# f1tenth/f1tenth_gym

Hardware: AMD Instinct MI355X
Metric: agent-steps/s (1080-beam scan + ST dynamics) (higher is better)
Workload: dtype f64

## Files before the change

### f1tenth_gym_amd/csrc/f110_hip.hip

```cpp
#include <hip/hip_runtime.h>
#include <rccl/rccl.h>

#include <dlfcn.h>

#include <algorithm>
#include <chrono>
#include <cmath>
#include <cstdarg>
#include <cstdio>
#include <cstdlib>
#include <cstring>
#include <map>
#include <mutex>
#include <new>
#include <set>
#include <string>
#include <vector>

#include "../../include/f110.h"
#include "f110_kernels.hpp"
#include "f110_devmem.hpp"

using devmem::DevArena;
using devmem::DevBuf;
// ... 2590 lines not shown
    double *d = reinterpret_cast<double *>(base + ((ints * 4 + 63) / 64) * 64);
    t.state = d;            d += 7 * N;
    t.steer_buf = d;        d += 2 * N;
    t.scan_pose = d;        d += 3 * N;
    t.snap_pose = d;        d += 3 * N;
    t.dir_start = d;        d += N;
    t.ray_hdr = reinterpret_cast<RayHdr *>(d);
    t.tasks_per_agent = ((uint32_t)h->k.num_beams + 63u) / 64u;
    return F110_OK;
}

static int step_tiny(f110_sim *h, hipStream_t st, const double *d_actions, const StepRequest &rq, bool &host_written)
{
    TRY(tiny_setup(h));
    const int N = h->N, A = h->cfg.num_agents;
    AgentArrays dev = h->dev;
    dev.agent_begin = 0;
    dev.agent_count = N;
    dev.sched_count_zero = nullptr;
    RayJob j{};
    j.noise = h->dev.noise;
    j.ttc_side_max = h->ttc_side_max;
    j.ttc_k = h->dev.ttc_thresh * (1.0 + 1e-9) * h->ttc_cos_max;
    j.beam_cos = h->dev.beam_cos;
    j.side_dist = h->dev.side_dist;
    j.ttc_thresh = h->dev.ttc_thresh;
    j.k_cold = cold_consts(h);
    if (!j.k_cold) return fail(h, F110_ERR_HIP, "f110_step_device: constant upload failed");
    h->tiny.tasks_per_agent = ((uint32_t)h->k.num_beams + 63u) / 64u;
    h->tiny.trace = kExperimental ? reinterpret_cast<unsigned long long *>(h->exp.tiny_trace) : nullptr;
    h->tiny.act_inline = 0;
    if (rq.tiny_actions && N <= kTinyMaxAgents) {
        std::memcpy(h->tiny.act, rq.tiny_actions, sizeof(double) * 2 * (size_t)N);
        h->tiny.act_inline = 1;
    }
    h->tiny.start_word = nullptr;
    h->tiny.skip = kExperimental ? (h->exp.tiny_start_probe == 2 ? 1 : (h->exp.tiny_general_tail ? 2 : 0)) : 0;
    if (kExperimental && h->exp.tiny_start_probe && h->hb_seq_host && rq.seq) {
        void *p = nullptr;
        TRY(map_host_ptr(h, h->hb_seq_host, &p, "completion word"));
        h->tiny.start_word = reinterpret_cast<unsigned long long *>(p) + 1;
        h->tiny.start_seq = h->hb_seq;
    }
    const dim3 grid(((unsigned)N * h->tiny.tasks_per_agent + 3u) / 4u), block(256);
    const bool host = !dev.reseat_poses && (A == 2 ? rq.fuse : rq.hb != nullptr), solo = host && A != 2;
    host_written = host;
// ... 12 lines not shown
    if (A == 2) {
        if (host) { if (ident) TINY(true, true, true); else TINY(true, false, true); }
        else { if (ident) TINY(true, true, false); else TINY(true, false, false); }
    } else {
        if (host) { if (ident) TINY(false, true, true); else TINY(false, false, true); }
        else { if (ident) TINY(false, true, false); else TINY(false, false, false); }
    }
#undef TINY
    h->last_launches = 1;
    if (h->track_on) {
        TRY(track_launch(h, st, kTrackPost, 0, N));
        h->last_launches += 2;
    }
    return F110_OK;
}

static int step_range(f110_sim *h, hipStream_t st, int begin, int count, const double *d_actions, int collide_mode, hipEvent_t *ev, const StepRequest &rq,
                      bool &host_written)
{
    const int N = h->N, A = h->cfg.num_agents, B = h->k.num_beams;
    AgentArrays dev = h->dev;
    dev.agent_begin = begin;
    dev.agent_count = count;
    const bool multi = A > 1;
    const ScanKind scan = pick_scan(h, begin, count);
    if (h->track_on) TRY(track_launch(h, st, kTrackHead, begin, count));
    dev.sched_count_zero = scan == SCAN_AGENT_SCHED ? h->d_tcount + (h->task_epoch & 1u) : nullptr;
    if (dev.noise_rng && (dev.noise_rng == 2 || h->noise_ub >= (long long)dev.noise_rows)) {
        const int apb = dev.noise_rng == 2 ? 16 : 64;
        hipLaunchKernelGGL(k_noise_rows, dim3((count + apb - 1) / apb), dim3(256), 0, st, dev, h->noise_gen, B, apb);
    }
    if (ev) HIPCHK(h, hipEventRecord(ev[0], st));
    bool fused_integrate = false;
#ifdef F110_EXPERIMENTAL
    if (multi && collide_mode == 1 && A == 2) {
        hipLaunchKernelGGL(k_integrate<2>, grid1d(count, 64), dim3(64), 0, st, dev, h->k, d_actions);
        fused_integrate = true;
    } else if (multi && collide_mode == 1 && A == 4) {
        hipLaunchKernelGGL(k_integrate<4>, grid1d(count, 64), dim3(64), 0, st, dev, h->k, d_actions);
        fused_integrate = true;
    }
#endif
    if (!fused_integrate) {
        bool duo = true;
        bool fan = h->dev.integrator == F110_INTEGRATOR_RK4 && count <= kFanMaxAgents;
#ifdef F110_EXPERIMENTAL
// ... 10 lines not shown
    const bool multi_in_finalize = multi && collide_mode == 3 && A > 2 && A <= kMaxAgentsMulti && (begin % A) == 0 && (count % A) == 0;
    const bool no_collide_launch = fused_integrate || pair_in_finalize || multi_in_finalize;
    const bool side_collide = multi && !no_collide_launch && !(kExperimental && collide_mode == 2);
    if (multi && !no_collide_launch) {
        if (side_collide) {
            HIPCHK(h, hipEventRecord(h->ev_integrated, st));
            HIPCHK(h, hipStreamWaitEvent(h->side_stream, h->ev_integrated, 0));
            hipLaunchKernelGGL(k_collide, grid1d(count, 64), dim3(64), 0, h->side_stream, dev, B);
            HIPCHK(h, hipEventRecord(h->ev_collided, h->side_stream));
        } else {
            hipLaunchKernelGGL(k_collide, grid1d(count, 64), dim3(64), 0, st, dev, B);
        }
    }
    if (ev) HIPCHK(h, hipEventRecord(ev[1], st));
    {
        RayJob j{};
        j.n_rays = (uint32_t)N * (uint32_t)B;
        j.n_poses = N;
        j.pose_x = h->dev.scan_pose;
        j.pose_y = h->dev.scan_pose + N;
        j.dir_start = h->dev.dir_start;
        j.ranges = h->dev.scans;
        j.hdr = h->dev.ray_hdr;
        j.noise = h->dev.noise;
        j.ttc_side_max = h->ttc_side_max;
        j.ttc_k = h->dev.ttc_thresh * (1.0 + 1e-9) * h->ttc_cos_max;
        j.beam_cos = h->dev.beam_cos;
        j.side_dist = h->dev.side_dist;
        j.wall_flag = h->dev.in_collision;
        j.ttc_thresh = h->dev.ttc_thresh;
        j.div_magic = h->step_magic;
        j.div_shift = h->step_shift;
        j.lookups_total = h->lookups_on ? h->d_lookups : nullptr;
        j.path_stats = h->path_stats_on ? h->d_path_stats : nullptr;
#ifdef F110_EXPERIMENTAL
        j.trace = reinterpret_cast<unsigned long long *>(h->exp.scan_trace);
#endif
        j.k_cold = cold_consts(h);
        if (!j.k_cold) return fail(h, F110_ERR_HIP, "f110_step_device: constant upload failed");
        j.order = (h->multi_map && begin == 0 && count == N) ? h->d_scan_order : nullptr;
        const bool cnt = j.lookups_total != nullptr;
        const bool env_order = h->scan_env_order && !h->multi_map && (scan == SCAN_AGENT || scan == SCAN_AGENT_SCHED);
        auto agent_grid = [&](uint32_t tpa, dim3 &grid, uint32_t &wpb, int tpw) {
            (void)rays_grid(j, h->scan_block, tpw);
            j.n_tasks = (uint32_t)count * tpa;
            j.first_pose = (uint32_t)begin;
            j.agents_per_env = (env_order && A > 1 && begin % A == 0 && count % A == 0 && scan_task_inv_ok(tpa, (uint32_t)A)) ? (uint32_t)A : 1u;
            j.agents_inv = scan_task_inv(j.agents_per_env);
            wpb = (uint32_t)h->scan_block / 64u;
// ... 3170 lines not shown
```

### f1tenth_gym_amd/csrc/f110_kernels.hpp

```cpp
#pragma once

#include <hip/hip_runtime.h>
#include <stdint.h>

#include "f110_math.hpp"
#include "f110_rng.hpp"

using namespace f110;

struct RayHdr {
    double x, y;
    double start;
    double vel;
    double d0;
    int32_t noise_row;
    int32_t map_slot;
    int32_t pad_hdr;
    int32_t i0;
    int32_t n_dirs;
    int32_t fast;
};
static_assert(sizeof(RayHdr) == 64, "RayHdr is read as 16-byte scalar loads");

struct AgentArrays {
    int32_t n_agents_total;
    int32_t agents_per_env;
    int32_t agent_begin, agent_count;
    double *state;
    double *steer_buf;
    int32_t *buf_cnt;
    double *scan_pose;
    double *snap_pose;
    double *dir_start;
    RayHdr *ray_hdr;
    double *scans;
    double *collisions;
// ... 3 lines not shown
    unsigned long long *path_stats;
    const ScanConst *maps_full;
    const int32_t *env_map;
    const double *reseat_poses;
    int32_t *reseat_count;
    int32_t reseat_ego, pad_reseat;
    uint32_t *sched_count_zero;
    int32_t *opp_window;
    double *opp_verts;
    const double *params;
    int32_t params_per_agent, pad_params;
    const double *noise;
    int32_t noise_rng, pad_rng;
    U128 *rng_state;
    const U128 *rng_seed;
    const U128 *rng_rowstate;
    U128 rng_inc;
    const double *scan_angles, *beam_cos, *side_dist;
    int32_t noise_rows, integrator;
    double time_step, lidar_dist, ttc_thresh, angle_inc;
    double box_length, box_width;
    const struct FusedHost *fused_host;
    unsigned long long fused_seq;
};

__device__ __forceinline__ VehicleParams load_params(const double *p)
{
    VehicleParams vp;
#pragma unroll
    for (int i = 0; i < NPARAMS; ++i) vp.v[i] = p[i];
    return vp;
}

struct EpisodeArrays {
    int32_t ego_idx, pad;
    double timestep;
    double *start_poses;
    double *rot;
    double *current_time;
    uint8_t *near_start;
    double *toggle;
    double *lap_count;
    double *lap_time;
    uint8_t *done;
    uint8_t *checkpoint;
};
// ... 89 lines not shown
        }
        int ref_lo, ref_hi, lo, hi;
        box_vertices(ox, oy, oth, blen, bwid, other);
        int32_t *win = a.opp_window + ((size_t)i * A + j) * 4;
        opponent_beam_window(mx, my, mth, other, ox, oy, disc_r, a.scan_angles, B, a.angle_inc, ref_lo, ref_hi, lo, hi);
        win[0] = lo;
        win[1] = hi;
        opponent_beam_window(mx, my, 0.0, other, ox, oy, disc_r, a.scan_angles, B, a.angle_inc, ref_lo, ref_hi, lo, hi);
        win[2] = lo;
        win[3] = hi;
        double *ov = a.opp_verts + ((size_t)i * A + j) * 8;
#pragma unroll
        for (int c = 0; c < 8; ++c) ov[c] = other[c];
    }
    a.collisions[i] = hit ? 1.0 : 0.0;
    a.collision_idx[i] = (double)partner;
}

__device__ __forceinline__ RayHdr make_ray_hdr(const AgentArrays &a, const ScanConst &k, int i, const double *st, const double *sp, double start)
{
    RayHdr hd;
    ScanConst kr = k;
    kr.table = k.table_rm;
    hd.x = sp[0];
    hd.y = sp[1];
    hd.start = start;
    hd.vel = st[3];
    hd.map_slot = a.env_map ? a.env_map[i / a.agents_per_env] : 0;
    hd.pad_hdr = 0;
    const ScanConst *km = a.env_map ? a.maps_full + hd.map_slot : &kr;
    int r0, c0;
    hd.d0 = sample_distance<LAYOUT_ROWMAJOR, false, false>(*km, nullptr, sp[0], sp[1], r0, c0);
    int row = -1;
    if (a.noise_rng) {
        row = a.step_count[i];
        if (a.noise_rng == 2 || row >= a.noise_rows) row = -2;
    } else if (a.noise_rows > 0) {
        row = a.step_count[i];
        if (row >= a.noise_rows) row %= a.noise_rows;
    }
    hd.noise_row = row;
    hd.i0 = beam_dir_index(k, start, 0);
    hd.fast = 0;
    if (km->pad) {
        double ux, uy;
        padded_position<false>(*km, sp[0], sp[1], ux, uy);
        hd.fast = padded_start_ok(*km, ux, uy) ? 1 : 0;
    }
    hd.n_dirs = 0;
    if (k.theta_inc < 1.0) {
        int span = beam_dir_index(k, start, k.num_beams - 1) - hd.i0;
        if (span < 0) span += k.theta_dis;
        hd.n_dirs = span + 1;
    }
    return hd;
}

__device__ __forceinline__ void integrate_store_columns(const AgentArrays &a, int i, int N, const double *st, double b0, double b1, int cnt, const double *sp,
                                                        double start)
{
#pragma unroll
    for (int c = 0; c < 7; ++c) a.state[(size_t)c * N + i] = st[c];
    a.steer_buf[i] = b0;
    a.steer_buf[(size_t)N + i] = b1;
    a.buf_cnt[i] = cnt;
    a.scan_pose[i] = sp[0];
    a.scan_pose[(size_t)N + i] = sp[1];
    a.scan_pose[2 * (size_t)N + i] = sp[2];
    a.snap_pose[i] = st[0];
    a.snap_pose[(size_t)N + i] = st[1];
// ... 207 lines not shown
    uint32_t *count_w;
    uint32_t cap, thr;
    const void *reserved_r[8];
    uint32_t reserved_rcap, reserved_rthr;
};

struct RayJob {
    uint32_t n_rays;
    uint32_t n_tasks;
    uint32_t tasks_per_wave;
    int32_t n_poses;
    uint32_t div_magic, div_shift;
    int32_t pad_dir, dir_stride;
    const void *reserved_dir_ranges;
    uint32_t first_pose, agents_per_env;
    unsigned long long *lookups_total;
    TaskSched sched;
    uint32_t epoch_r, epoch_w, long_blocks, agents_inv;
    uint32_t *env_done;
    uint32_t tasks_per_env, long_prio;
    uint32_t long_rev, pad_rev;
    unsigned long long *trace;
    const uint32_t *order;
    const void *reserved_win[2];
    uint32_t reserved_win_pitch, pad_win;
    const double *pose_x, *pose_y, *dir_start;
    double *ranges;
    const RayHdr *hdr;
    const double *noise;
    const double *beam_cos, *side_dist;
    int32_t *wall_flag;
    double ttc_thresh;
    double ttc_side_max, ttc_k;
    int32_t *hit_rc;
    unsigned long long *lookups;
    unsigned long long *path_stats;
    const ScanConst *k_cold;
};

__device__ __forceinline__ int uniform_i32(int v) { return __builtin_amdgcn_readfirstlane(v); }
__device__ __forceinline__ double uniform_f64(double v)
{
    const int lo = __builtin_amdgcn_readfirstlane(__double2loint(v));
    const int hi = __builtin_amdgcn_readfirstlane(__double2hiint(v));
    return __hiloint2double(hi, lo);
}

struct LaneHdr {
    double x, y, start, vel, d0;
    int row, map_slot, i0, n_dirs, fast;
};

__device__ __forceinline__ LaneHdr load_lane_hdr(const RayHdr *hdr, uint32_t p)
{
    LaneHdr o;
    const uint32_t p0 = __builtin_amdgcn_readfirstlane(p);
    if (__ballot(p != p0) == 0ull) {
        typedef const __attribute__((address_space(4))) RayHdr *chdr_t;
        const chdr_t h0 = (chdr_t)(hdr) + p0;
        o.x = uniform_f64(h0->x);
        o.y = uniform_f64(h0->y);
        o.start = uniform_f64(h0->start);
        o.vel = uniform_f64(h0->vel);
        o.d0 = uniform_f64(h0->d0);
        o.row = uniform_i32(h0->noise_row);
        o.map_slot = uniform_i32(h0->map_slot);
        o.i0 = uniform_i32(h0->i0);
        o.n_dirs = uniform_i32(h0->n_dirs);
        o.fast = uniform_i32(h0->fast);
    } else {
        const RayHdr hd = hdr[p];
        o.x = hd.x; o.y = hd.y; o.start = hd.start; o.vel = hd.vel; o.d0 = hd.d0; o.row = hd.noise_row;
        o.map_slot = hd.map_slot; o.i0 = hd.i0; o.n_dirs = hd.n_dirs;
        o.fast = hd.fast;
    }
    return o;
}

struct RayJob;
__device__ __forceinline__ void finish_beam(const RayJob &j, uint32_t B, uint32_t p, int b, uint32_t ray, double r,
                                            int row, double vel);
__device__ __forceinline__ void finish_beam_with(const RayJob &j, uint32_t p, int b, uint32_t ray, double r, double vel);

__device__ __forceinline__ void wave_add_lookups(unsigned long long *total, uint32_t mine)
{
    for (int off = 32; off; off >>= 1) mine += __shfl_xor(mine, off);
    if ((threadIdx.x & 63u) == 0u) atomicAdd(total, (unsigned long long)mine);
}

template <int LAYOUT, bool POW2, bool IDENT, bool WANT_CELL>
__device__ __forceinline__ double trace_from_first(const ScanConst &k, const ScanConst *k_cold, const double *lut, double x, double y,
                                                   bool fast, double c, double s, double d0, int &hr, int &hc, int &nl,
                                                   int &path)
{
    if (LAYOUT == LAYOUT_PADDED) {
        double r = 0.;
        bool exact = !fast;
        if (fast) {
            double ux, uy, cux, cuy;
            padded_position<IDENT>(k, x, y, ux, uy);
            padded_rate<IDENT>(k, c, s, cux, cuy);
            exact = !march_padded<WANT_CELL>(k, ux, uy, cux, cuy, d0, r, hr, hc, nl);
        }
        path = fast ? (exact ? 1 : 0) : 2;
        if (exact) r = march_exact_cold<IDENT>(k_cold, x, y, c, s, d0, hr, hc, nl);
        return r;
    }
    path = 2;
    return march_from_first<LAYOUT, POW2, IDENT>(k, lut, x, y, c, s, d0, hr, hc, nl);
}

template <int LAYOUT, bool POW2, bool IDENT, bool STEP>
__global__ void __launch_bounds__(256) k_scan_rays(RayJob j, ScanConst k)
{
    const double *lut_lds = nullptr;
    const uint32_t B = (uint32_t)k.num_beams;
    const uint32_t tpw = j.tasks_per_wave;
    const uint32_t lane = threadIdx.x & 63u;
    uint32_t blk = blockIdx.x;
    {
        const uint32_t nb = gridDim.x, q = nb >> 3, rem = nb & 7u, x = blk & 7u, i = blk >> 3;
        blk = (x < rem ? x * (q + 1u) : rem * (q + 1u) + (x - rem) * q) + i;
    }
    const uint32_t wave = (blk * blockDim.x + threadIdx.x) >> 6;
    uint32_t nl_acc = 0;
    for (uint32_t t = 0; t < tpw; ++t) {
        const uint32_t task = wave * tpw + t;
        if (task >= j.n_tasks) break;
        const uint32_t ray = task * 64u + lane;
        if (ray >= j.n_rays) break;
        const uint32_t p = j.div_magic ? (__umulhi(ray, j.div_magic) >> j.div_shift) : ray / B;
        const int b = (int)(ray - p * B);
        int hr, hc, nl, path;
        double r;
        if (STEP) {
            const LaneHdr hd = load_lane_hdr(j.hdr, p);
            hr = -1;
            hc = -1;
            const double2 cs = k.cs[beam_dir_index(k, hd.start, b)];
            r = trace_from_first<LAYOUT, POW2, IDENT, false>(k, j.k_cold, lut_lds, hd.x, hd.y, hd.fast != 0, cs.x, cs.y, hd.d0, hr, hc, nl, path);
            nl_acc += (uint32_t)nl;
            finish_beam(j, B, p, b, ray, r, hd.row, hd.vel);
            continue;
        } else {
            const double2 cs = k.cs[beam_dir_index(k, j.dir_start[p], b)];
            const double x = j.pose_x[p], y = j.pose_y[p];
            const double d0 = sample_distance<LAYOUT, POW2, IDENT>(k, lut_lds, x, y, hr, hc);
            bool fast = false;
            if (LAYOUT == LAYOUT_PADDED) {
                double ux, uy;
                padded_position<IDENT>(k, x, y, ux, uy);
                fast = padded_start_ok(k, ux, uy);
            }
            r = trace_from_first<LAYOUT, POW2, IDENT, true>(k, j.k_cold, lut_lds, x, y, fast, cs.x, cs.y, d0, hr, hc, nl, path);
            if (j.path_stats) atomicAdd(&j.path_stats[path], 1ull);
            if (j.hit_rc) {
                j.hit_rc[(size_t)ray * 2] = hr;
                j.hit_rc[(size_t)ray * 2 + 1] = hc;
            }
            if (j.lookups) atomicAdd(&j.lookups[p], (unsigned long long)nl);
        }
        j.ranges[ray] = r;
    }
    if (STEP && j.lookups_total) wave_add_lookups(j.lookups_total, nl_acc);
}

struct MapFast {
    const double *pad;
    double pad_cx, pad_cy;
    double pad_axx, pad_axy, pad_ayx, pad_ayy;
    uint32_t pad_row_bytes;
    int32_t pad_max_samples;
};
static_assert(sizeof(MapFast) == 64, "MapFast is read as one 64-byte scalar load");

__device__ __forceinline__ void load_map_fast(ScanConst &km, const MapFast *__restrict__ maps_fast, int slot)
{
    typedef const __attribute__((address_space(4))) MapFast *cmap_t;
    const cmap_t m0 = (cmap_t)(maps_fast) + slot;
    const uint64_t pa = (uint64_t)m0->pad;
    km.pad = (const double *)(((uint64_t)(uint32_t)uniform_i32((int)(pa >> 32)) << 32) | (uint32_t)uniform_i32((int)pa));
    km.pad_cx = uniform_f64(m0->pad_cx);
    km.pad_cy = uniform_f64(m0->pad_cy);
    km.pad_axx = uniform_f64(m0->pad_axx);
    km.pad_axy = uniform_f64(m0->pad_axy);
    km.pad_ayx = uniform_f64(m0->pad_ayx);
    km.pad_ayy = uniform_f64(m0->pad_ayy);
    km.pad_row_bytes = uniform_i32((int)m0->pad_row_bytes);
    km.pad_max_samples = uniform_i32(m0->pad_max_samples);
}

#ifndef F110_SCAN_WAVES_EXPR
#define F110_SCAN_WAVES_EXPR 8
#endif
template <bool PER_ENV_MAP, bool IDENT, bool COUNT, bool SCHED = false, bool ENVCNT = false, bool ENV_ORDER = false>
__global__ void __launch_bounds__(256) __attribute__((amdgpu_waves_per_eu(F110_SCAN_WAVES_EXPR))) k_scan_rays_agent(RayJob j, ScanConst k, const MapFast *__restrict__ maps_fast,
                                                          const ScanConst *__restrict__ maps_full, uint32_t tasks_per_agent)
{
    static_assert(!(ENV_ORDER && PER_ENV_MAP), "a per-env order and the env order exclude each other");
    const uint32_t B = (uint32_t)k.num_beams;
    uint32_t tpw = j.tasks_per_wave;
    const uint32_t lane = threadIdx.x & 63u;
    uint32_t blk = blockIdx.x;
    typedef const __attribute__((address_space(4))) uint32_t *cu32_t;
    bool long_pass = false;
    uint32_t long_task = 0;
#ifdef F110_EXPERIMENTAL
    const unsigned long long trace_begin = j.trace ? wall_clock64() : 0ull;
    unsigned long long trace_loop = 0ull, trace_hdr = 0ull, trace_ops = 0ull, trace_marched = 0ull;
    uint32_t trace_samples = 0;
#endif
    if (SCHED) {
        if (blk < j.long_blocks) {
            const TaskSched &sc = j.sched;
            const uint32_t wl = __builtin_amdgcn_readfirstlane((blk * blockDim.x + threadIdx.x) >> 6);
            uint32_t cnt = *(cu32_t)sc.count_r;
            cnt = cnt < sc.cap ? cnt : sc.cap;
            if (wl >= cnt) return;
            long_pass = true;
            long_task = ((cu32_t)sc.list_r)[j.long_rev ? cnt - 1u - wl : wl];
            tpw = 1u;
            if (j.long_prio) __builtin_amdgcn_s_setprio(3);
// ... 6 lines not shown
        blk = (x < rem ? x * (q + 1u) : rem * (q + 1u) + (x - rem) * q) + i;
    }
    const uint32_t wave = (blk * blockDim.x + threadIdx.x) >> 6;
    uint32_t nl_acc = 0;
    ScanConst km = k;
    const ScanConst *cold = j.k_cold;
    int cur_slot = -1;
    double held = 0.0;
    int held_row = -1;
    uint32_t held_sec = 0;
#ifdef F110_EXPERIMENTAL
    if (j.trace) trace_loop = wall_clock64();
#endif
    for (uint32_t t = 0; t < tpw; ++t) {
        const uint32_t task = __builtin_amdgcn_readfirstlane(long_pass ? long_task : wave * tpw + t);
        if (task >= j.n_tasks) break;
        uint32_t pl, sec = 0;
        if (!ENV_ORDER) pl = task / tasks_per_agent;
        else scan_task_agent(task, tasks_per_agent, j.agents_per_env, j.agents_inv, pl, sec);
        const uint32_t p = (PER_ENV_MAP && j.order) ? ((cu32_t)j.order)[pl] : j.first_pose + pl;
        const uint32_t stamp = (SCHED && !long_pass) ? ((cu32_t)j.sched.flags_r)[task] : 0u;
        typedef const __attribute__((address_space(4))) RayHdr *chdr_t;
        const chdr_t h0 = (chdr_t)(j.hdr) + p;
        const double x = uniform_f64(h0->x), y = uniform_f64(h0->y), start = uniform_f64(h0->start);
        const double vel = uniform_f64(h0->vel), d0 = uniform_f64(h0->d0);
        const int row = uniform_i32(h0->noise_row), slot = uniform_i32(h0->map_slot), fast = uniform_i32(h0->fast);
#ifdef F110_EXPERIMENTAL
        if (j.trace && trace_hdr == 0ull) trace_hdr = wall_clock64();
#endif
        if (SCHED && !long_pass && stamp == j.epoch_r) continue;
        const bool load_nz = !ENV_ORDER || row < 0 || row != held_row || sec != held_sec;
        if (ENV_ORDER) {
            held_row = row;
            held_sec = sec;
        }
        const int b = (int)((ENV_ORDER ? sec : task - pl * tasks_per_agent) * 64u + lane);
        if (b >= (int)B) continue;
        if (PER_ENV_MAP && slot != cur_slot) {
            cold = maps_full + slot;
            load_map_fast(km, maps_fast, slot);
            cur_slot = slot;
        }
        const double *nrow = row >= 0 ? j.noise + (size_t)row * B : j.ranges + (size_t)p * B;
        if (ENV_ORDER && load_nz) held = row != -1 ? nrow[b] : 0.0;
        const double nz = ENV_ORDER ? held : (row != -1 ? nrow[b] : 0.0);
        double2 cs = k.cs[beam_dir_index(k, start, b)];
#ifdef F110_EXPERIMENTAL
        if (j.trace && trace_ops == 0ull) {
            asm volatile("" : "+v"(cs.x), "+v"(cs.y));
            trace_ops = wall_clock64();
        }
#endif
        int hr = -1, hc = -1, nl = 0;
        double r = 0.;
        bool exact = fast == 0;
        if (fast) {
            double ux, uy, cux, cuy;
            padded_position<IDENT>(km, x, y, ux, uy);
            padded_rate<IDENT>(km, cs.x, cs.y, cux, cuy);
            exact = !march_padded<false>(km, ux, uy, cux, cuy, d0, r, hr, hc, nl);
        }
        if (exact) r = march_exact_cold<IDENT>(cold, x, y, cs.x, cs.y, d0, hr, hc, nl);
        if (COUNT) nl_acc += (uint32_t)nl;
#ifdef F110_EXPERIMENTAL
        if (j.trace) {
            asm volatile("" : "+v"(r));
            trace_marched = wall_clock64();
        }
        if (j.trace) {
            int m = 0;
            for (int bit = 1 << 10; bit; bit >>= 1)
                if (__ballot(nl >= (m | bit)) != 0ull) m |= bit;
            trace_samples += (uint32_t)m;
        }
#endif
        if (SCHED) {
            const TaskSched &sc = j.sched;
            if (__ballot(nl > (int)sc.thr) != 0ull && lane == 0u) {
                const uint32_t pos = atomicAdd(sc.count_w, 1u);
                if (pos < sc.cap) {
                    sc.list_w[pos] = task;
                    sc.flags_w[task] = j.epoch_w;
                }
            }
        }
        finish_beam_with(j, p, b, p * B + (uint32_t)b, row != -1 ? r + nz : r, vel);
        if (ENVCNT && lane == 0u) {
            const uint32_t env = p / (j.tasks_per_env / tasks_per_agent);
            const uint32_t old = __hip_atomic_fetch_add(j.env_done + env, 1u, __ATOMIC_RELAXED, __HIP_MEMORY_SCOPE_AGENT);
            if (old + 1u == j.tasks_per_env) __hip_atomic_store(j.env_done + env, 0u, __ATOMIC_RELAXED, __HIP_MEMORY_SCOPE_AGENT);
        }
    }
    if (COUNT) wave_add_lookups(j.lookups_total, nl_acc);
#ifdef F110_EXPERIMENTAL
    if (j.trace && lane == 0u) {
        uint32_t hw_id, xcc_id;
        asm volatile("s_getreg_b32 %0, hwreg(HW_REG_HW_ID)" : "=s"(hw_id));
        asm volatile("s_getreg_b32 %0, hwreg(HW_REG_XCC_ID)" : "=s"(xcc_id));
        unsigned long long *rec = j.trace + 8ull * ((blockIdx.x * blockDim.x + threadIdx.x) >> 6);
        rec[0] = trace_begin;
        rec[1] = wall_clock64();
        rec[2] = (unsigned long long)hw_id | ((unsigned long long)xcc_id << 32);
        rec[3] = (unsigned long long)trace_samples | ((unsigned long long)(long_pass ? 1u : 0u) << 32);
        rec[4] = trace_loop;
        rec[5] = trace_hdr;
        rec[6] = trace_ops;
        rec[7] = trace_marched;
    }
#endif
}


__device__ __forceinline__ void finish_beam_with(const RayJob &j, uint32_t p, int b, uint32_t ray, double r, double vel)
{
    if (vel != 0.0 && !(r > j.ttc_side_max + j.ttc_k * fabs(vel)) &&
        ttc_beam_hit(r, j.side_dist[b], vel, j.beam_cos[b], j.ttc_thresh))
        j.wall_flag[p] = 1;
    j.ranges[ray] = r;
}

__device__ __forceinline__ void finish_beam(const RayJob &j, uint32_t B, uint32_t p, int b, uint32_t ray, double r,
                                            int row, double vel)
{
    if (row >= 0)
        r += j.noise[(size_t)row * B + b];
    else if (row == -2)
        r += j.ranges[ray];
    finish_beam_with(j, p, b, ray, r, vel);
}

#ifndef F110_DIRS_WAVES_EXPR
#define F110_DIRS_WAVES_EXPR 8
#endif
template <bool PER_ENV_MAP, bool IDENT, bool COUNT>
__global__ void __launch_bounds__(256) __attribute__((amdgpu_waves_per_eu(F110_DIRS_WAVES_EXPR))) k_scan_dirs_agent(RayJob j, ScanConst k, const MapFast *__restrict__ maps_fast,
                                                          const ScanConst *__restrict__ maps_full, uint32_t tasks_per_agent)
{
    const uint32_t B = (uint32_t)k.num_beams;
    const uint32_t tpw = j.tasks_per_wave;
    const uint32_t lane = threadIdx.x & 63u;
    uint32_t blk = blockIdx.x;
    {
        const uint32_t nb = gridDim.x, q = nb >> 3, rem = nb & 7u, x = blk & 7u, i = blk >> 3;
        blk = (x < rem ? x * (q + 1u) : rem * (q + 1u) + (x - rem) * q) + i;
    }
    const uint32_t wave = (blk * blockDim.x + threadIdx.x) >> 6;
    uint32_t nl_acc = 0;
    ScanConst km = k;
    const ScanConst *cold = j.k_cold;
    int cur_slot = -1;
    for (uint32_t t = 0; t < tpw; ++t) {
        const uint32_t task = __builtin_amdgcn_readfirstlane(wave * tpw + t);
        if (task >= j.n_tasks) break;
        const uint32_t pl = task / tasks_per_agent;
        typedef const __attribute__((address_space(4))) uint32_t *cu32_t;
        const uint32_t p = (PER_ENV_MAP && j.order) ? ((cu32_t)j.order)[pl] : j.first_pose + pl;
        const int s0 = (int)((task - pl * tasks_per_agent) * 64u);
        typedef const __attribute__((address_space(4))) RayHdr *chdr_t;
        const chdr_t h0 = (chdr_t)(j.hdr) + p;
        const int n_dirs = uniform_i32(h0->n_dirs);
        if (s0 >= n_dirs) continue;
        const double x = uniform_f64(h0->x), y = uniform_f64(h0->y), start = uniform_f64(h0->start);
        const double vel = uniform_f64(h0->vel), d0 = uniform_f64(h0->d0);
        const int row = uniform_i32(h0->noise_row), fast = uniform_i32(h0->fast), i0 = uniform_i32(h0->i0);
        if (PER_ENV_MAP) {
            const int slot = uniform_i32(h0->map_slot);
            if (slot != cur_slot) {
                cold = maps_full + slot;
                load_map_fast(km, maps_fast, slot);
                cur_slot = slot;
            }
        }
        auto rel_of = [&](int b) {
            int rr = beam_dir_index(k, start, b) - i0;
            return rr < 0 ? rr + k.theta_dis : rr;
        };
        int b0 = 0;
        if (s0 > 0) {
            b0 = (int)ceil(((double)s0 - (start - floor(start))) / k.theta_inc) - 2;
            b0 = b0 < 0 ? 0 : (b0 >= (int)B ? (int)B - 1 : b0);
            b0 = __builtin_amdgcn_readfirstlane(b0);
            while (b0 > 0 && rel_of(b0 - 1) >= s0) --b0;
            while (b0 < (int)B && rel_of(b0) < s0) ++b0;
        }
        constexpr int kPre = 3;
        const double *nrow = row >= 0 ? j.noise + (size_t)row * B : j.ranges + (size_t)p * B;
        bool pre_in[kPre];
        int pre_src[kPre];
        double pre_nz[kPre];
#pragma unroll
        for (int q = 0; q < kPre; ++q) {
            const int b = b0 + (int)lane + 64 * q;
            bool in = b < (int)B;
            int src = 0;
            if (in) {
                src = rel_of(b) - s0;
                in = src < 64;
            }
            pre_in[q] = in;
            pre_src[q] = src;
            pre_nz[q] = (in && row != -1) ? nrow[b] : 0.0;
        }
        double r_dir = 0.;
        if (s0 + (int)lane < n_dirs) {
            int didx = i0 + s0 + (int)lane;
            if (didx >= k.theta_dis) didx -= k.theta_dis;
            const double2 cs = k.cs[didx];
            int hr = -1, hc = -1, nl;
            bool exact = fast == 0;
            if (fast) {
                double ux, uy, cux, cuy;
                padded_position<IDENT>(km, x, y, ux, uy);
                padded_rate<IDENT>(km, cs.x, cs.y, cux, cuy);
                exact = !march_padded<false>(km, ux, uy, cux, cuy, d0, r_dir, hr, hc, nl);
            }
            if (exact) r_dir = march_exact_cold<IDENT>(cold, x, y, cs.x, cs.y, d0, hr, hc, nl);
            if (COUNT) nl_acc += (uint32_t)nl;
        }
        bool more = true;
#pragma unroll
        for (int q = 0; q < kPre; ++q) {
            if (more) {
                const int b = b0 + (int)lane + 64 * q;
                const double r = __shfl(r_dir, pre_in[q] ? pre_src[q] : 0);
                if (pre_in[q]) finish_beam_with(j, p, b, p * B + (uint32_t)b, row != -1 ? r + pre_nz[q] : r, vel);
                if (__ballot(!pre_in[q]) != 0ull) more = false;
            }
        }
        for (int b = b0 + (int)lane + 64 * kPre; more; b += 64) {
            bool in = b < (int)B;
            int src = 0;
            if (in) {
                src = rel_of(b) - s0;
                in = src < 64;
            }
            const double r = __shfl(r_dir, in ? src : 0);
            if (in) finish_beam(j, B, p, b, p * B + (uint32_t)b, r, row, vel);
            if (__ballot(!in) != 0ull) more = false;
        }
    }
    if (COUNT) wave_add_lookups(j.lookups_total, nl_acc);
}


struct NoiseGen {
    const uint64_t *zk;
    const double *zw, *zf;
    const U128 *ja, *jg;
    double scale;
};

__device__ __forceinline__ void noise_row_wave(const NoiseGen &g, U128 &state, const U128 inc, double *__restrict__ out, int B)
{
    const int lane = (int)(threadIdx.x & 63u);
    const ZigTables zt = {g.zk, g.zw, g.zf};
    const U128 aj = g.ja[lane + 1];
    const U128 gi = mul128(g.jg[lane + 1], inc);
    const uint64_t below = (1ull << lane) - 1ull;
    int produced = 0, skip = 0;
    U128 s = state;
// ... 1384 lines not shown
        advance_vehicle(st, b0, b1, cnt, act.x, act.y, vp, a.time_step, a.integrator, a.lidar_dist, sp);
        const double start = scan_start_index(k, sp[2]);
        const RayHdr hd = make_ray_hdr(a, k, i, st, sp, start);
#ifdef F110_EXPERIMENTAL
        if (ctl.trace) {
            double probe = hd.d0;
            asm volatile("" : "+v"(probe));
        }
#endif
        TINY_STAMP(1);
        if (sub == 0u && lane == 0u) {
            integrate_store_columns(sh, i, N, st, b0, b1, cnt, sp, start);
            sh.ray_hdr[i] = hd;
        }
        const int b = (int)(sub * 64u + lane);
        if (b < B) {
            const int row = hd.noise_row;
            const double nz = row >= 0 ? j.noise[(size_t)row * B + b] : 0.0;
            const double2 cs = k.cs[beam_dir_index(k, start, b)];
            int hr = -1, hc = -1, nl = 0;
            double r = 0.;
            bool exact = hd.fast == 0;
            if (hd.fast) {
                double ux, uy, cux, cuy;
                padded_position<IDENT>(k, hd.x, hd.y, ux, uy);
                padded_rate<IDENT>(k, cs.x, cs.y, cux, cuy);
                exact = !march_padded<false>(k, ux, uy, cux, cuy, hd.d0, r, hr, hc, nl);
            }
            if (exact) r = march_exact_cold<IDENT>(j.k_cold, hd.x, hd.y, cs.x, cs.y, hd.d0, hr, hc, nl);
            if (row != -1) r += nz;
            if (hd.vel != 0.0 && !(r > j.ttc_side_max + j.ttc_k * fabs(hd.vel)) && ttc_beam_hit(r, j.side_dist[b], hd.vel, j.beam_cos[b], j.ttc_thresh))
                sh.in_collision[i] = 1;
            a.scans[(size_t)i * B + b] = r;
        }
    }
    TINY_STAMP(2);
    __builtin_amdgcn_s_waitcnt(0);
    __syncthreads();
    TINY_STAMP(3);
    if (threadIdx.x == 0) {
        __threadfence();
        const unsigned int prev = __hip_atomic_fetch_add(ctl.done, 1u, __ATOMIC_ACQ_REL, __HIP_MEMORY_SCOPE_AGENT);
        s_last = prev == gridDim.x - 1u ? 1 : 0;
        if (s_last) __hip_atomic_store(ctl.done, 0u, __ATOMIC_RELAXED, __HIP_MEMORY_SCOPE_AGENT);
    }
    __syncthreads();
    if (!s_last) return;
    __threadfence();
    TINY_STAMP(4);
    TINY_STAMP(5);
    if (PAIR) {
        if (N == 2 && ctl.skip != 2) {
            finalize_duo_tiny<HOST>(sh, B, HOST ? ctl.host_scans : nullptr, ctl.fh);
            TINY_STAMP(6);
// ... 2390 lines not shown
__global__ void __launch_bounds__(256) k_pf_sense(PfJob j, ScanConst k, int ppw)
{
    __shared__ double s_term[256];
    const int P = j.sp.P, B = j.sp.B;
    const int tid = (int)threadIdx.x, q = tid / B, jb = tid - q * B;
    const long long total = (long long)j.count * P;
    const long long gp = (long long)blockIdx.x * ppw + q;
    const bool live = q < ppw && gp < total;
    const size_t G = (size_t)j.i0 * P + (size_t)(live ? gp : 0);
    double term = 0.0;
    if (live) {
        const int i = j.i0 + (int)(gp / P);
        const int n = j.agents ? j.agents[i] : i;
        const PfHdr hd = j.hdr[G];
        const int beam = j.sp.beam_first + jb * j.sp.beam_stride;
        const double z = j.scans[(size_t)n * j.num_beams + beam];
        const ScanConst *cold = j.maps + (j.env_map ? j.env_map[n / j.A] : 0);
        const ScanConst km = *cold;
        int di = beam_dir_index(k, hd.start, beam);
        di = di < 0 ? 0 : di;
        const double2 cs = k.cs[di];
        int hr = -1, hc = -1, nl, path;
        double r;
        if (km.pad)
            r = trace_from_first<LAYOUT_PADDED, false, false, false>(km, cold, nullptr, hd.x, hd.y, hd.fast != 0, cs.x, cs.y, hd.d0, hr, hc, nl, path);
        else
            r = march_from_first<LAYOUT_ROWMAJOR, false, false>(km, nullptr, hd.x, hd.y, cs.x, cs.y, hd.d0, hr, hc, nl);
        if (j.expect) j.expect[G * B + jb] = r;
        term = pf_term(j.sp, z, r);
    }
    s_term[tid] = term;
    __syncthreads();
    if (live && jb == 0) j.logw[G] = pf_logw(j.sp, s_term + tid, B);
}

inline int pf_group_lanes(int P)
{
    const int need = P < 256 ? P : 256;
    int gs = 16;
    while (gs < need) gs <<= 1;
    return gs;
}

constexpr int kPfSlots = 8;

__global__ void __launch_bounds__(256) k_pf_update(PfJob j, int GS)
{
    extern __shared__ double s_pf_upd[];
    __shared__ double s_slot[16][kPfSlots];
// ... 51 lines not shown
```

### f1tenth_gym_amd/csrc/f110_math.hpp

```cpp
#pragma once

#include <hip/hip_runtime.h>
#include <math.h>
#include <stdint.h>

#define F110_HD __host__ __device__ __forceinline__

namespace f110 {

constexpr double kPi = 3.14159265358979323846;
constexpr double kTwoPi = 2.0 * kPi;

enum { P_MU = 0, P_CSF, P_CSR, P_LF, P_LR, P_H, P_M, P_I, P_SMIN, P_SMAX, P_SVMIN, P_SVMAX,
       P_VSWITCH, P_AMAX, P_VMIN, P_VMAX, P_WIDTH, P_LENGTH, NPARAMS };

struct VehicleParams {
    double v[NPARAMS];
};

F110_HD void cos_sin(double a, double &c, double &s)
{
#if defined(__HIP_DEVICE_COMPILE__)
    sincos(a, &s, &c);
#else
// ... 485 lines not shown
    } else {
        ux = fma(x, k.pad_axx, fma(y, k.pad_axy, k.pad_cx));
        uy = fma(y, k.pad_ayy, fma(x, k.pad_ayx, k.pad_cy));
    }
}

template <bool IDENT>
F110_HD void padded_rate(const ScanConst &k, double c, double s, double &cux, double &cuy)
{
    if (IDENT) {
        cux = c * k.inv_res;
        cuy = s * k.inv_res;
    } else {
        cux = fma(c, k.pad_axx, s * k.pad_axy);
        cuy = fma(s, k.pad_ayy, c * k.pad_ayx);
    }
}

F110_HD bool padded_start_ok(const ScanConst &k, double ux, double uy)
{
    return (ux >= k.pad_lo) & (ux <= k.pad_hi_x) & (uy >= k.pad_lo) & (uy <= k.pad_hi_y);
}

template <bool WANT_CELL>
F110_HD bool march_padded(const ScanConst &k, double ux, double uy, double cux, double cuy, double d, double &range,
                          int &hit_r, int &hit_c, int &lookups)
{
    double total = d;
    int n = 1;
    double lim = k.max_range;
    const char *base = reinterpret_cast<const char *>(k.pad);
    while ((d > k.eps) & (total <= lim)) {
        ux = fma(d, cux, ux);
        uy = fma(d, cuy, uy);
        const uint32_t wx = low_word(ux + kFixBig);
        const uint32_t wy = low_word(uy + kFixBig);
        uint32_t off = mul24(wy >> kFixFracBits, (uint32_t)k.pad_row_bytes) + ((wx >> kFixFracBits) << 3);
        if (WANT_CELL) {
            hit_c = (int)(wx >> kFixFracBits);
            hit_r = (int)(wy >> kFixFracBits);
        }
        const bool edge = mul24(wx & 0xffffu, wy & 0xffffu) == 0u;
        if (__builtin_expect(any_lane(edge), 0)) {
            const bool near = (fabs(ux - rint(ux)) < kPadGuard) | (fabs(uy - rint(uy)) < kPadGuard);
            lim = (edge & near) ? -1.0 : lim;
            const int fc = (int)floor(ux), fr = (int)floor(uy);
            const uint32_t off_floor = mul24((uint32_t)fr, (uint32_t)k.pad_row_bytes) + ((uint32_t)fc << 3);
            off = edge ? off_floor : off;
            if (WANT_CELL) {
                hit_c = edge ? fc : hit_c;
                hit_r = edge ? fr : hit_r;
            }
        }
        F110_MARCH_OFFSET_HOOK(off);
        d = *reinterpret_cast<const double *>(base + off);
        total += d;
        ++n;
    }
    if (WANT_CELL && n > 1) {
        hit_c -= k.pad_border;
        hit_r -= k.pad_border;
        if (hit_c < 0 || hit_c >= k.width || hit_r < 0 || hit_r >= k.height) {
            hit_r = -1;
            hit_c = -1;
        }
    }
    lookups = n;
    range = (total > k.max_range) ? k.max_range : total;
    return !((lim < 0.0) | (n > k.pad_max_samples));
}


template <bool IDENT>
F110_HD double march_exact_cold(const ScanConst *kc_in, double x, double y, double c, double s, double d, int &hit_r,
                                int &hit_c, int &lookups)
{
    const volatile ScanConst *kc = kc_in;
    double total = d;
    int n = 1;
    while (d > kc->eps && total <= kc->max_range) {
// ... 48 lines not shown
    }
    int idx = (int)t;
    return idx >= k.theta_dis ? k.theta_dis - 1 : idx;
}

F110_HD uint32_t scan_task_inv(uint32_t A) { return A > 1u ? (uint32_t)(0x100000000ull / A) + 1u : 0u; }
F110_HD bool scan_task_inv_ok(uint32_t tpa, uint32_t A) { return (unsigned long long)tpa * A * A <= 0x100000000ull; }
F110_HD void scan_task_agent(uint32_t task, uint32_t tpa, uint32_t A, uint32_t inv_A, uint32_t &agent, uint32_t &sector)
{
    const uint32_t tpe = tpa * A, env = task / tpe, rem = task - env * tpe;
    sector = inv_A ? (uint32_t)(((unsigned long long)rem * inv_A) >> 32) : rem;
    agent = env * A + (rem - sector * A);
}

F110_HD bool ttc_beam_hit(double range, double side_distance, double vel, double beam_cos, double thresh)
{
    const double proj_vel = vel * beam_cos;
    const double num = range - side_distance;
    const double a = fabs(num), b = fabs(proj_vel);
    if (a < (thresh * (1.0 - 1e-12)) * b) return (num == 0.0) || ((num > 0.0) == (proj_vel > 0.0));
    if (a > (thresh * (1.0 + 1e-12)) * b) return false;
    const double ttc = num / proj_vel;
    return (ttc < thresh) && (ttc >= 0.0);
}

F110_HD double edge_range(double ox, double oy, double v3x, double v3y, double vax, double vay,
                          double vbx, double vby)
{
    const double v1x = ox - vax, v1y = oy - vay;
    const double v2x = vbx - vax, v2y = vby - vay;
    const double denom = v2x * v3x + v2y * v3y;
    double distance = INFINITY;
    if (fabs(denom) > 0.0) {
        const double d1 = (v2x * v1y - v2y * v1x) / denom;
        const double d2 = (v1x * v3x + v1y * v3y) / denom;
        if (d1 >= 0.0 && d2 >= 0.0 && d2 <= 1.0) distance = d1;
    } else {
        const double bax = vax - ox, bay = vay - oy;
        const double cax = ox - vbx, cay = oy - vby;
        if (fabs(bax * cay - bay * cax) < 1e-8) {
            const double da = sqrt(bax * bax + bay * bay);
            const double dbx = vbx - ox, dby = vby - oy;
            const double db = sqrt(dbx * dbx + dby * dby);
            distance = da < db ? da : db;
        }
    }
// ... 1280 lines not shown
```

Measured before the change: 105.7 million.

## Precompute padded start coords and TTC cutoff in ray headers, trim march counting

The per-agent ray header now stores the padded-grid start position and a precomputed TTC cutoff instead of the world position and velocity. Scan kernels skip the per-lane padded_position transform and the per-beam cutoff arithmetic. They fetch world pose and velocity from cold arrays only on the rare exact-march or TTC-candidate paths. The padded march also gets a variant that drops sample counting when no counters are needed. The cost is extra indirect loads on slow paths and more template variants.

```diff
diff --git a/f1tenth_gym_amd/csrc/f110_hip.hip b/f1tenth_gym_amd/csrc/f110_hip.hip
--- a/f1tenth_gym_amd/csrc/f110_hip.hip
+++ b/f1tenth_gym_amd/csrc/f110_hip.hip
@@ -2636,6 +2636,8 @@
     j.noise = h->dev.noise;
     j.ttc_side_max = h->ttc_side_max;
     j.ttc_k = h->dev.ttc_thresh * (1.0 + 1e-9) * h->ttc_cos_max;
+    dev.ttc_side_max = j.ttc_side_max;
+    dev.ttc_k = j.ttc_k;
     j.beam_cos = h->dev.beam_cos;
     j.side_dist = h->dev.side_dist;
     j.ttc_thresh = h->dev.ttc_thresh;
@@ -2694,6 +2696,8 @@
     AgentArrays dev = h->dev;
     dev.agent_begin = begin;
     dev.agent_count = count;
+    dev.ttc_side_max = h->ttc_side_max;
+    dev.ttc_k = h->dev.ttc_thresh * (1.0 + 1e-9) * h->ttc_cos_max;
     const bool multi = A > 1;
     const ScanKind scan = pick_scan(h, begin, count);
     if (h->track_on) TRY(track_launch(h, st, kTrackHead, begin, count));
@@ -2750,9 +2754,12 @@
         j.dir_start = h->dev.dir_start;
         j.ranges = h->dev.scans;
         j.hdr = h->dev.ray_hdr;
+        j.pose_cold = h->dev.scan_pose;
+        j.vel_cold = h->dev.state + 3 * (size_t)N;
+        j.cold_pitch = (uint32_t)N;
         j.noise = h->dev.noise;
-        j.ttc_side_max = h->ttc_side_max;
-        j.ttc_k = h->dev.ttc_thresh * (1.0 + 1e-9) * h->ttc_cos_max;
+        j.ttc_side_max = dev.ttc_side_max;
+        j.ttc_k = dev.ttc_k;
         j.beam_cos = h->dev.beam_cos;
         j.side_dist = h->dev.side_dist;
         j.wall_flag = h->dev.in_collision;
diff --git a/f1tenth_gym_amd/csrc/f110_kernels.hpp b/f1tenth_gym_amd/csrc/f110_kernels.hpp
--- a/f1tenth_gym_amd/csrc/f110_kernels.hpp
+++ b/f1tenth_gym_amd/csrc/f110_kernels.hpp
@@ -9,9 +9,9 @@
 using namespace f110;
 
 struct RayHdr {
-    double x, y;
+    double sx, sy;
     double start;
-    double vel;
+    double ttc_cut;
     double d0;
     int32_t noise_row;
     int32_t map_slot;
@@ -61,6 +61,7 @@
     double box_length, box_width;
     const struct FusedHost *fused_host;
     unsigned long long fused_seq;
+    double ttc_side_max, ttc_k;
 };
 
 __device__ __forceinline__ VehicleParams load_params(const double *p)
@@ -196,10 +197,10 @@
     RayHdr hd;
     ScanConst kr = k;
     kr.table = k.table_rm;
-    hd.x = sp[0];
-    hd.y = sp[1];
+    hd.sx = sp[0];
+    hd.sy = sp[1];
     hd.start = start;
-    hd.vel = st[3];
+    hd.ttc_cut = ttc_cutoff(st[3], a.ttc_side_max, a.ttc_k);
     hd.map_slot = a.env_map ? a.env_map[i / a.agents_per_env] : 0;
     hd.pad_hdr = 0;
     const ScanConst *km = a.env_map ? a.maps_full + hd.map_slot : &kr;
@@ -218,8 +219,13 @@
     hd.fast = 0;
     if (km->pad) {
         double ux, uy;
-        padded_position<false>(*km, sp[0], sp[1], ux, uy);
+        if (!a.env_map && k.ident_rot) padded_position<true>(*km, sp[0], sp[1], ux, uy);
+        else padded_position<false>(*km, sp[0], sp[1], ux, uy);
         hd.fast = padded_start_ok(*km, ux, uy) ? 1 : 0;
+        if (hd.fast) {
+            hd.sx = ux;
+            hd.sy = uy;
+        }
     }
     hd.n_dirs = 0;
     if (k.theta_inc < 1.0) {
@@ -473,8 +479,9 @@
     uint32_t long_rev, pad_rev;
     unsigned long long *trace;
     const uint32_t *order;
-    const void *reserved_win[2];
-    uint32_t reserved_win_pitch, pad_win;
+    const double *pose_cold;
+    const double *vel_cold;
+    uint32_t cold_pitch, pad_win;
     const double *pose_x, *pose_y, *dir_start;
     double *ranges;
     const RayHdr *hdr;
@@ -498,7 +505,7 @@
 }
 
 struct LaneHdr {
-    double x, y, start, vel, d0;
+    double sx, sy, start, ttc_cut, d0;
     int row, map_slot, i0, n_dirs, fast;
 };
 
@@ -509,10 +516,10 @@
     if (__ballot(p != p0) == 0ull) {
         typedef const __attribute__((address_space(4))) RayHdr *chdr_t;
         const chdr_t h0 = (chdr_t)(hdr) + p0;
-        o.x = uniform_f64(h0->x);
-        o.y = uniform_f64(h0->y);
+        o.sx = uniform_f64(h0->sx);
+        o.sy = uniform_f64(h0->sy);
         o.start = uniform_f64(h0->start);
-        o.vel = uniform_f64(h0->vel);
+        o.ttc_cut = uniform_f64(h0->ttc_cut);
         o.d0 = uniform_f64(h0->d0);
         o.row = uniform_i32(h0->noise_row);
         o.map_slot = uniform_i32(h0->map_slot);
@@ -521,7 +528,7 @@
         o.fast = uniform_i32(h0->fast);
     } else {
         const RayHdr hd = hdr[p];
-        o.x = hd.x; o.y = hd.y; o.start = hd.start; o.vel = hd.vel; o.d0 = hd.d0; o.row = hd.noise_row;
+        o.sx = hd.sx; o.sy = hd.sy; o.start = hd.start; o.ttc_cut = hd.ttc_cut; o.d0 = hd.d0; o.row = hd.noise_row;
         o.map_slot = hd.map_slot; o.i0 = hd.i0; o.n_dirs = hd.n_dirs;
         o.fast = hd.fast;
     }
@@ -530,8 +537,8 @@
 
 struct RayJob;
 __device__ __forceinline__ void finish_beam(const RayJob &j, uint32_t B, uint32_t p, int b, uint32_t ray, double r,
-                                            int row, double vel);
-__device__ __forceinline__ void finish_beam_with(const RayJob &j, uint32_t p, int b, uint32_t ray, double r, double vel);
+                                            int row, double ttc_cut);
+__device__ __forceinline__ void finish_beam_with(const RayJob &j, uint32_t p, int b, uint32_t ray, double r, double ttc_cut);
 
 __device__ __forceinline__ void wave_add_lookups(unsigned long long *total, uint32_t mine)
 {
@@ -539,26 +546,35 @@
     if ((threadIdx.x & 63u) == 0u) atomicAdd(total, (unsigned long long)mine);
 }
 
-template <int LAYOUT, bool POW2, bool IDENT, bool WANT_CELL>
-__device__ __forceinline__ double trace_from_first(const ScanConst &k, const ScanConst *k_cold, const double *lut, double x, double y,
+__device__ __forceinline__ void scan_world_position(const RayJob &j, uint32_t p, double &x, double &y)
+{
+    x = j.pose_cold[p];
+    y = j.pose_cold[(size_t)j.cold_pitch + p];
+}
+
+template <int LAYOUT, bool POW2, bool IDENT, bool WANT_CELL, typename World>
+__device__ __forceinline__ double trace_from_first(const ScanConst &k, const ScanConst *k_cold, const double *lut, double sx, double sy,
                                                    bool fast, double c, double s, double d0, int &hr, int &hc, int &nl,
-                                                   int &path)
+                                                   int &path, World world)
 {
     if (LAYOUT == LAYOUT_PADDED) {
         double r = 0.;
         bool exact = !fast;
         if (fast) {
-            double ux, uy, cux, cuy;
-            padded_position<IDENT>(k, x, y, ux, uy);
+            double cux, cuy;
             padded_rate<IDENT>(k, c, s, cux, cuy);
-            exact = !march_padded<WANT_CELL>(k, ux, uy, cux, cuy, d0, r, hr, hc, nl);
+            exact = !march_padded<WANT_CELL>(k, sx, sy, cux, cuy, d0, r, hr, hc, nl);
         }
         path = fast ? (exact ? 1 : 0) : 2;
-        if (exact) r = march_exact_cold<IDENT>(k_cold, x, y, c, s, d0, hr, hc, nl);
+        if (exact) {
+            double x = sx, y = sy;
+            if (fast) world(x, y);
+            r = march_exact_cold<IDENT>(k_cold, x, y, c, s, d0, hr, hc, nl);
+        }
         return r;
     }
     path = 2;
-    return march_from_first<LAYOUT, POW2, IDENT>(k, lut, x, y, c, s, d0, hr, hc, nl);
+    return march_from_first<LAYOUT, POW2, IDENT>(k, lut, sx, sy, c, s, d0, hr, hc, nl);
 }
 
 template <int LAYOUT, bool POW2, bool IDENT, bool STEP>
@@ -589,21 +605,23 @@
             hr = -1;
             hc = -1;
             const double2 cs = k.cs[beam_dir_index(k, hd.start, b)];
-            r = trace_from_first<LAYOUT, POW2, IDENT, false>(k, j.k_cold, lut_lds, hd.x, hd.y, hd.fast != 0, cs.x, cs.y, hd.d0, hr, hc, nl, path);
+            r = trace_from_first<LAYOUT, POW2, IDENT, false>(k, j.k_cold, lut_lds, hd.sx, hd.sy, hd.fast != 0, cs.x, cs.y, hd.d0, hr, hc, nl, path,
+                                                             [&](double &wx, double &wy) { scan_world_position(j, p, wx, wy); });
             nl_acc += (uint32_t)nl;
-            finish_beam(j, B, p, b, ray, r, hd.row, hd.vel);
+            finish_beam(j, B, p, b, ray, r, hd.row, hd.ttc_cut);
             continue;
         } else {
             const double2 cs = k.cs[beam_dir_index(k, j.dir_start[p], b)];
             const double x = j.pose_x[p], y = j.pose_y[p];
             const double d0 = sample_distance<LAYOUT, POW2, IDENT>(k, lut_lds, x, y, hr, hc);
             bool fast = false;
+            double ux = x, uy = y;
             if (LAYOUT == LAYOUT_PADDED) {
-                double ux, uy;
                 padded_position<IDENT>(k, x, y, ux, uy);
                 fast = padded_start_ok(k, ux, uy);
             }
-            r = trace_from_first<LAYOUT, POW2, IDENT, true>(k, j.k_cold, lut_lds, x, y, fast, cs.x, cs.y, d0, hr, hc, nl, path);
+            r = trace_from_first<LAYOUT, POW2, IDENT, true>(k, j.k_cold, lut_lds, fast ? ux : x, fast ? uy : y, fast, cs.x, cs.y, d0, hr, hc, nl, path,
+                                                            [&](double &wx, double &wy) { wx = x; wy = y; });
             if (j.path_stats) atomicAdd(&j.path_stats[path], 1ull);
             if (j.hit_rc) {
                 j.hit_rc[(size_t)ray * 2] = hr;
@@ -649,6 +667,11 @@
                                                           const ScanConst *__restrict__ maps_full, uint32_t tasks_per_agent)
 {
     static_assert(!(ENV_ORDER && PER_ENV_MAP), "a per-env order and the env order exclude each other");
+#ifdef F110_EXPERIMENTAL
+    constexpr bool kCountSamples = true;
+#else
+    constexpr bool kCountSamples = COUNT || SCHED;
+#endif
     const uint32_t B = (uint32_t)k.num_beams;
     uint32_t tpw = j.tasks_per_wave;
     const uint32_t lane = threadIdx.x & 63u;
@@ -701,8 +724,8 @@
         const uint32_t stamp = (SCHED && !long_pass) ? ((cu32_t)j.sched.flags_r)[task] : 0u;
         typedef const __attribute__((address_space(4))) RayHdr *chdr_t;
         const chdr_t h0 = (chdr_t)(j.hdr) + p;
-        const double x = uniform_f64(h0->x), y = uniform_f64(h0->y), start = uniform_f64(h0->start);
-        const double vel = uniform_f64(h0->vel), d0 = uniform_f64(h0->d0);
+        const double sx = uniform_f64(h0->sx), sy = uniform_f64(h0->sy), start = uniform_f64(h0->start);
+        const double ttc_cut = uniform_f64(h0->ttc_cut), d0 = uniform_f64(h0->d0);
         const int row = uniform_i32(h0->noise_row), slot = uniform_i32(h0->map_slot), fast = uniform_i32(h0->fast);
 #ifdef F110_EXPERIMENTAL
         if (j.trace && trace_hdr == 0ull) trace_hdr = wall_clock64();
@@ -734,12 +757,15 @@
         double r = 0.;
         bool exact = fast == 0;
         if (fast) {
-            double ux, uy, cux, cuy;
-            padded_position<IDENT>(km, x, y, ux, uy);
+            double cux, cuy;
             padded_rate<IDENT>(km, cs.x, cs.y, cux, cuy);
-            exact = !march_padded<false>(km, ux, uy, cux, cuy, d0, r, hr, hc, nl);
-        }
-        if (exact) r = march_exact_cold<IDENT>(cold, x, y, cs.x, cs.y, d0, hr, hc, nl);
+            exact = !march_padded<false, kCountSamples>(km, sx, sy, cux, cuy, d0, r, hr, hc, nl);
+        }
+        if (exact) {
+            double x = sx, y = sy;
+            if (fast) scan_world_position(j, p, x, y);
+            r = march_exact_cold<IDENT>(cold, x, y, cs.x, cs.y, d0, hr, hc, nl);
+        }
         if (COUNT) nl_acc += (uint32_t)nl;
 #ifdef F110_EXPERIMENTAL
         if (j.trace) {
@@ -763,7 +789,7 @@
                 }
             }
         }
-        finish_beam_with(j, p, b, p * B + (uint32_t)b, row != -1 ? r + nz : r, vel);
+        finish_beam_with(j, p, b, p * B + (uint32_t)b, row != -1 ? r + nz : r, ttc_cut);
         if (ENVCNT && lane == 0u) {
             const uint32_t env = p / (j.tasks_per_env / tasks_per_agent);
             const uint32_t old = __hip_atomic_fetch_add(j.env_done + env, 1u, __ATOMIC_RELAXED, __HIP_MEMORY_SCOPE_AGENT);
@@ -790,22 +816,23 @@
 }
 
 
-__device__ __forceinline__ void finish_beam_with(const RayJob &j, uint32_t p, int b, uint32_t ray, double r, double vel)
-{
-    if (vel != 0.0 && !(r > j.ttc_side_max + j.ttc_k * fabs(vel)) &&
-        ttc_beam_hit(r, j.side_dist[b], vel, j.beam_cos[b], j.ttc_thresh))
-        j.wall_flag[p] = 1;
+__device__ __forceinline__ void finish_beam_with(const RayJob &j, uint32_t p, int b, uint32_t ray, double r, double ttc_cut)
+{
+    if (!(r > ttc_cut)) {
+        const double vel = j.vel_cold[p];
+        if (vel != 0.0 && ttc_beam_hit(r, j.side_dist[b], vel, j.beam_cos[b], j.ttc_thresh)) j.wall_flag[p] = 1;
+    }
     j.ranges[ray] = r;
 }
 
 __device__ __forceinline__ void finish_beam(const RayJob &j, uint32_t B, uint32_t p, int b, uint32_t ray, double r,
-                                            int row, double vel)
+                                            int row, double ttc_cut)
 {
     if (row >= 0)
         r += j.noise[(size_t)row * B + b];
     else if (row == -2)
         r += j.ranges[ray];
-    finish_beam_with(j, p, b, ray, r, vel);
+    finish_beam_with(j, p, b, ray, r, ttc_cut);
 }
 
 #ifndef F110_DIRS_WAVES_EXPR
@@ -839,8 +866,8 @@
         const chdr_t h0 = (chdr_t)(j.hdr) + p;
         const int n_dirs = uniform_i32(h0->n_dirs);
         if (s0 >= n_dirs) continue;
-        const double x = uniform_f64(h0->x), y = uniform_f64(h0->y), start = uniform_f64(h0->start);
-        const double vel = uniform_f64(h0->vel), d0 = uniform_f64(h0->d0);
+        const double sx = uniform_f64(h0->sx), sy = uniform_f64(h0->sy), start = uniform_f64(h0->start);
+        const double ttc_cut = uniform_f64(h0->ttc_cut), d0 = uniform_f64(h0->d0);
         const int row = uniform_i32(h0->noise_row), fast = uniform_i32(h0->fast), i0 = uniform_i32(h0->i0);
         if (PER_ENV_MAP) {
             const int slot = uniform_i32(h0->map_slot);
@@ -885,15 +912,18 @@
             int didx = i0 + s0 + (int)lane;
             if (didx >= k.theta_dis) didx -= k.theta_dis;
             const double2 cs = k.cs[didx];
-            int hr = -1, hc = -1, nl;
+            int hr = -1, hc = -1, nl = 0;
             bool exact = fast == 0;
             if (fast) {
-                double ux, uy, cux, cuy;
-                padded_position<IDENT>(km, x, y, ux, uy);
+                double cux, cuy;
                 padded_rate<IDENT>(km, cs.x, cs.y, cux, cuy);
-                exact = !march_padded<false>(km, ux, uy, cux, cuy, d0, r_dir, hr, hc, nl);
+                exact = !march_padded<false, COUNT>(km, sx, sy, cux, cuy, d0, r_dir, hr, hc, nl);
             }
-            if (exact) r_dir = march_exact_cold<IDENT>(cold, x, y, cs.x, cs.y, d0, hr, hc, nl);
+            if (exact) {
+                double x = sx, y = sy;
+                if (fast) scan_world_position(j, p, x, y);
+                r_dir = march_exact_cold<IDENT>(cold, x, y, cs.x, cs.y, d0, hr, hc, nl);
+            }
             if (COUNT) nl_acc += (uint32_t)nl;
         }
         bool more = true;
@@ -902,7 +932,7 @@
             if (more) {
                 const int b = b0 + (int)lane + 64 * q;
                 const double r = __shfl(r_dir, pre_in[q] ? pre_src[q] : 0);
-                if (pre_in[q]) finish_beam_with(j, p, b, p * B + (uint32_t)b, row != -1 ? r + pre_nz[q] : r, vel);
+                if (pre_in[q]) finish_beam_with(j, p, b, p * B + (uint32_t)b, row != -1 ? r + pre_nz[q] : r, ttc_cut);
                 if (__ballot(!pre_in[q]) != 0ull) more = false;
             }
         }
@@ -914,7 +944,7 @@
                 in = src < 64;
             }
             const double r = __shfl(r_dir, in ? src : 0);
-            if (in) finish_beam(j, B, p, b, p * B + (uint32_t)b, r, row, vel);
+            if (in) finish_beam(j, B, p, b, p * B + (uint32_t)b, r, row, ttc_cut);
             if (__ballot(!in) != 0ull) more = false;
         }
     }
@@ -2345,14 +2375,13 @@
             double r = 0.;
             bool exact = hd.fast == 0;
             if (hd.fast) {
-                double ux, uy, cux, cuy;
-                padded_position<IDENT>(k, hd.x, hd.y, ux, uy);
+                double cux, cuy;
                 padded_rate<IDENT>(k, cs.x, cs.y, cux, cuy);
-                exact = !march_padded<false>(k, ux, uy, cux, cuy, hd.d0, r, hr, hc, nl);
+                exact = !march_padded<false, false>(k, hd.sx, hd.sy, cux, cuy, hd.d0, r, hr, hc, nl);
             }
-            if (exact) r = march_exact_cold<IDENT>(j.k_cold, hd.x, hd.y, cs.x, cs.y, hd.d0, hr, hc, nl);
+            if (exact) r = march_exact_cold<IDENT>(j.k_cold, sp[0], sp[1], cs.x, cs.y, hd.d0, hr, hc, nl);
             if (row != -1) r += nz;
-            if (hd.vel != 0.0 && !(r > j.ttc_side_max + j.ttc_k * fabs(hd.vel)) && ttc_beam_hit(r, j.side_dist[b], hd.vel, j.beam_cos[b], j.ttc_thresh))
+            if (!(r > hd.ttc_cut) && st[3] != 0.0 && ttc_beam_hit(r, j.side_dist[b], st[3], j.beam_cos[b], j.ttc_thresh))
                 sh.in_collision[i] = 1;
             a.scans[(size_t)i * B + b] = r;
         }
@@ -4789,9 +4818,12 @@
         const double2 cs = k.cs[di];
         int hr = -1, hc = -1, nl, path;
         double r;
-        if (km.pad)
-            r = trace_from_first<LAYOUT_PADDED, false, false, false>(km, cold, nullptr, hd.x, hd.y, hd.fast != 0, cs.x, cs.y, hd.d0, hr, hc, nl, path);
-        else
+        if (km.pad) {
+            double sx = hd.x, sy = hd.y;
+            if (hd.fast) padded_position<false>(km, hd.x, hd.y, sx, sy);
+            r = trace_from_first<LAYOUT_PADDED, false, false, false>(km, cold, nullptr, sx, sy, hd.fast != 0, cs.x, cs.y, hd.d0, hr, hc, nl, path,
+                                                                     [&](double &wx, double &wy) { wx = hd.x; wy = hd.y; });
+        } else
             r = march_from_first<LAYOUT_ROWMAJOR, false, false>(km, nullptr, hd.x, hd.y, cs.x, cs.y, hd.d0, hr, hc, nl);
         if (j.expect) j.expect[G * B + jb] = r;
         term = pf_term(j.sp, z, r);
diff --git a/f1tenth_gym_amd/csrc/f110_math.hpp b/f1tenth_gym_amd/csrc/f110_math.hpp
--- a/f1tenth_gym_amd/csrc/f110_math.hpp
+++ b/f1tenth_gym_amd/csrc/f110_math.hpp
@@ -531,10 +531,11 @@
     return (ux >= k.pad_lo) & (ux <= k.pad_hi_x) & (uy >= k.pad_lo) & (uy <= k.pad_hi_y);
 }
 
-template <bool WANT_CELL>
+template <bool WANT_CELL, bool WANT_COUNT = true>
 F110_HD bool march_padded(const ScanConst &k, double ux, double uy, double cux, double cuy, double d, double &range,
                           int &hit_r, int &hit_c, int &lookups)
 {
+    constexpr bool kLaneCount = WANT_COUNT || WANT_CELL;
     double total = d;
     int n = 1;
     double lim = k.max_range;
@@ -565,6 +566,11 @@
         d = *reinterpret_cast<const double *>(base + off);
         total += d;
         ++n;
+        if (!kLaneCount && __builtin_expect(n > k.pad_max_samples, 0)) lim = -1.0;
+    }
+    if (!kLaneCount) {
+        range = (total > k.max_range) ? k.max_range : total;
+        return !(lim < 0.0);
     }
     if (WANT_CELL && n > 1) {
         hit_c -= k.pad_border;
@@ -659,6 +665,11 @@
     if (a > (thresh * (1.0 + 1e-12)) * b) return false;
     const double ttc = num / proj_vel;
     return (ttc < thresh) && (ttc >= 0.0);
+}
+
+F110_HD double ttc_cutoff(double vel, double side_max, double k)
+{
+    return vel != 0.0 ? side_max + k * fabs(vel) : -INFINITY;
 }
 
 F110_HD double edge_range(double ox, double oy, double v3x, double v3y, double vax, double vay,
```

Result: no change. 105.9 million (median of 5 runs) (+0.2%).
